# Bergvca/string_grouper

Measured on AMD Instinct MI355X. Metric: hot-path rows/sec (the device path of match_strings: tokenise + tf-idf + postings + SpGEMM-topn, inputs resident in HBM), 663k-name self-join ntop=10 min_sim=0.8; match_strings end to end: match_strings_rows_per_s, higher is better.
Workload: dtype f32

## Files before the change

string_grouper_amd/csrc/sg_spgemm_pruned.hip:

```cpp
#define SG_WATCH_NAME sg_debug_watch_pruned
#include "sg_k4_device.h"

#ifdef SG_DEBUG_WAVE_TIMES
__device__ unsigned long long sg_debug_wave_times[4 * 16384];
extern "C" int sg_debug_read_wave_times(unsigned long long *out, int clear) {
    if (hipMemcpyFromSymbol(out, HIP_SYMBOL(sg_debug_wave_times), sizeof(sg_debug_wave_times)) != hipSuccess) return 1;
    if (clear) {
        static unsigned long long zero[4 * 16384];
        if (hipMemcpyToSymbol(HIP_SYMBOL(sg_debug_wave_times), zero, sizeof(zero)) != hipSuccess) return 1;
    }
    return 0;
}
#endif

#ifndef SG_F64_STREAM_WAVES
#define SG_F64_STREAM_WAVES 4
#endif
#define SG_SCHED_FENCE() __builtin_amdgcn_sched_barrier(0)
#define SG_ROW_PARTS_LOG2 6
#define SG_ROW_PARTS 64u
#define SG_SURV_CAP 128

__device__ __forceinline__ uint64_t ballot64(bool p) { return __builtin_amdgcn_ballot_w64(p); }

template <typename T>
__device__ __forceinline__ T wave_shfl(T v, int src) {
    return __shfl(v, src, 64);
}

#define SG_HASH_SLOTS 128
#ifdef SG_HASH_FINE
__device__ __forceinline__ uint32_t term_hash(int k) { return (__umul24((uint32_t)k & 0xffffffu, 0x9E3779u) >> 15) & 127u; }
#else
__device__ __forceinline__ uint32_t term_hash(int k) { return (__umul24((uint32_t)k & 0xffffffu, 0x9E3779u) >> 15) & 124u; }
#endif

template <typename P>
__device__ __forceinline__ P *lds_object(uint32_t byte_addr) {
    typedef __attribute__((address_space(3))) P lds_t;
    return (P *)(lds_t *)(uintptr_t)byte_addr;
}

template <typename P>
__device__ __forceinline__ const __attribute__((address_space(1))) P *global_ptr(const void *p) {
    return (const __attribute__((address_space(1))) P *)(uintptr_t)p;
}
typedef uint32_t sg_u32x4 __attribute__((ext_vector_type(4)));
typedef uint32_t sg_u32x2 __attribute__((ext_vector_type(2)));
__device__ __forceinline__ uint4 load_global_u4(const void *base, size_t idx) {
    const sg_u32x4 v = global_ptr<sg_u32x4>(base)[idx];
    return make_uint4(v.x, v.y, v.z, v.w);
}
__device__ __forceinline__ uint2 load_global_u2(const void *base, size_t idx) {
    const sg_u32x2 v = global_ptr<sg_u32x2>(base)[idx];
    return make_uint2(v.x, v.y);
}

template <typename S>
__device__ __forceinline__ S load_launch_constants(const S *p) {
    static_assert(sizeof(S) % 4 == 0, "dwords");
    const uint64_t a = (uint64_t)(uintptr_t)p;
    const uint64_t u = ((uint64_t)(uint32_t)__builtin_amdgcn_readfirstlane((int)(uint32_t)(a >> 32)) << 32) |
                       (uint64_t)(uint32_t)__builtin_amdgcn_readfirstlane((int)(uint32_t)a);
    typedef const __attribute__((address_space(4))) uint32_t *const_words;
    const const_words w = (const_words)(uintptr_t)u;
    union {
        S s;
        uint32_t d[sizeof(S) / 4];
    } out = {};
#pragma unroll
    for (unsigned i = 0; i < sizeof(S) / 4; ++i) out.d[i] = w[i];
    return out.s;
}

template <typename T>
struct FwdRound;
template <>
struct FwdRound<float> {
    int k[8];
    float v[8];
    __device__ __forceinline__ void load(const void *fwd, uint32_t q, uint32_t last) {
#pragma unroll
        for (int e = 0; e < 4; ++e) {
            const uint4 w = load_global_u4(fwd, min((q >> 1) + e, last >> 1));
            k[2 * e] = (int)w.x;
            v[2 * e] = __uint_as_float(w.y);
            k[2 * e + 1] = (int)w.z;
            v[2 * e + 1] = __uint_as_float(w.w);
        }
    }
};
template <>
struct FwdRound<double> {
    int k[8];
    double v[8];
// ... 332 lines not shown
        c0 = surv[lane];
        k0 = (uint32_t)lane < n_clean ||
             __hip_atomic_exchange(&dt[((uint32_t)c0 * 2654435761u) >> 25], (uint32_t)c0, __ATOMIC_RELAXED,
                                   __HIP_MEMORY_SCOPE_WORKGROUP) != (uint32_t)c0;
    }
    if ((uint32_t)lane + 64u < n_surv) {
        c1 = surv[lane + 64];
        k1 = (uint32_t)lane + 64u < n_clean ||
             __hip_atomic_exchange(&dt[((uint32_t)c1 * 2654435761u) >> 25], (uint32_t)c1, __ATOMIC_RELAXED,
                                   __HIP_MEMORY_SCOPE_WORKGROUP) != (uint32_t)c1;
    }
    const uint64_t f0 = ballot64(k0), f1 = ballot64(k1);
    const uint32_t n0 = (uint32_t)__popcll(f0);
    __builtin_amdgcn_wave_barrier();
    if (k0) surv[__popcll(f0 & lanes_below)] = c0;
    if (k1) surv[n0 + __popcll(f1 & lanes_below)] = c1;
    __builtin_amdgcn_wave_barrier();
    FlushOut<T> out;
    out.top = top;
    out.n_surv = (uint32_t)__builtin_amdgcn_readfirstlane((int)(n0 + (uint32_t)__popcll(f1)));
    if (out.n_surv >= 63u) {
        out.top = drain_survivors<T, SYM, TILE_LOG2, WIDE, true>(nnz, thr, row, sc, pairs, top, out.n_surv);
        const uint32_t scored = out.n_surv < 64u ? out.n_surv : 64u;
        out.n_surv = (out.n_surv - scored) | (scored << 16);
    }
    return out;
}

template <typename T, int TILE_LOG2>
__device__ __noinline__ void emit_part_matches(const SgPairSink *__restrict__ pairs, T s, int c, int cnt, uint32_t row_out) {
    constexpr int TILE = 1 << TILE_LOG2;
    int *surv = lds_object<int>(TILE * 2 + 512 + 1024);
    const int lane = threadIdx.x;
    if (cnt <= 0) return;
    uint32_t pos = (uint32_t)surv[SG_SURV_CAP - 1];
    const SgPairSink pv = load_launch_constants(pairs);
    const uint32_t pair_chunks = pv.chunks;
    if (pos == SG_PAIR_NO_CHUNK || (pos & 511u) + (uint32_t)cnt > SG_PAIR_CHUNK) {
        uint32_t ch = 0;
        if (lane == 0) {
            if (pos != SG_PAIR_NO_CHUNK && (pos >> 9) < pair_chunks) {
                pv.d_chunk_count[pos >> 9] = pos & 511u;
                atomicAdd(pv.d_totals, (unsigned long long)(pos & 511u));
            }
            ch = atomicAdd(pv.d_chunks_used, 1u);
        }
        pos = (uint32_t)__builtin_amdgcn_readfirstlane((int)ch) << 9;
    }
    if ((pos >> 9) < pair_chunks) {
        if (lane < cnt) {
            const size_t o = (size_t)(pos >> 9) * SG_PAIR_CHUNK + (pos & 511u) + (uint32_t)lane;
            pv.d_i[o] = (uint32_t)c;
            pv.d_j[o] = row_out;
            reinterpret_cast<T *>(pv.d_s)[o] = s;
        }
        if (lane == 0) atomicAdd(&pv.d_row_count[row_out], (uint32_t)cnt);
    }
    __builtin_amdgcn_wave_barrier();
    if (lane == 0) surv[SG_SURV_CAP - 1] = (int)(pos + (uint32_t)cnt);
}

template <typename T, int TILE_LOG2, bool SYM, bool WIDE, int FOLD_LOG2, bool SHARE = false>
__global__ void __launch_bounds__(64, (sizeof(T) == 8 && FOLD_LOG2 > 0) ? SG_F64_STREAM_WAVES : 4)
spgemm_topn_pruned_kernel(const int64_t *__restrict__ a_indptr, const int32_t *__restrict__ a_indices,
                          const T *__restrict__ a_data, uint32_t n_left, const uint32_t *__restrict__ seg,
                          const uint32_t *__restrict__ ends, int32_t nt_pad, uint32_t n_terms,
                          const uint32_t *__restrict__ filt, int32_t n_tiles,
                          const SgScoreCtx *__restrict__ sc ,
                          int32_t keep, int32_t out_stride, T thr,
                          float s_budget , float norm_b ,
                          uint32_t freq_min ,
                          int32_t *__restrict__ out_cols, T *__restrict__ out_vals, int32_t *__restrict__ out_cnt,
                          uint32_t *row_counter, uint32_t *flagged_count, uint32_t *flagged_rows,
                          unsigned long long *stats ,
                          const SgPairSink *__restrict__ pairs ,
                          uint32_t pair_chunks ,
                          uint32_t sym_lo, uint32_t sym_hi ,
                          const uint32_t *__restrict__ row_list , const uint32_t *row_list_len,
                          const uint32_t *__restrict__ ends8 , int32_t nv_pad,
                          uint32_t null_off ,
                          uint32_t n_right ,
                          uint32_t *heavy_count, uint32_t *heavy_rows ,
                          uint32_t sym_step, uint32_t deal_floor ,
                          uint32_t part_cfg ) {
    constexpr int TILE = 1 << TILE_LOG2;
    constexpr int SLOTS = WIDE ? 2 : 1;
    constexpr int AB = TILE_LOG2 + 1;
    constexpr uint32_t ADDR_MASK = ((1u << AB) - 1u) & ~3u;
    constexpr int FB = AB + FOLD_LOG2;
    constexpr uint32_t BQ_BITS = 24 - FB;
    constexpr uint32_t BQ_MAX = (1u << BQ_BITS) - 1u;
    constexpr float SCALE = (float)(32768 >> FOLD_LOG2);
    extern __shared__ __attribute__((aligned(16))) unsigned char smem[];
    int *hk = reinterpret_cast<int *>(smem + TILE * 2);
    T *ha = reinterpret_cast<T *>(smem + TILE * 2 + 512);
    int *surv = reinterpret_cast<int *>(smem + TILE * 2 + 512 + 1024);
    uint4 *tab_v = reinterpret_cast<uint4 *>(smem);
    const int lane = threadIdx.x;
    for (int x = lane; x < TILE * 2 / 16; x += 64) tab_v[x] = make_uint4(0, 0, 0, 0);
    if (SYM && lane == 0) surv[SG_SURV_CAP - 1] = (int)SG_PAIR_NO_CHUNK;
    if (FOLD_LOG2 > 0 && lane == 0) surv[SG_SURV_CAP - 2] = 0;
    const uint64_t lanes_below = (1ull << lane) - 1ull;
    unsigned long long st_rows = 0, st_post = 0, st_surv = 0;
    auto tab_at = [&](uint32_t byte_addr) {
        typedef __attribute__((address_space(3))) uint32_t lds_u32;
        return (uint32_t *)(lds_u32 *)(uintptr_t)byte_addr;
    };
    auto filt_at = [&](uint32_t byte_off) {
        return *reinterpret_cast<const uint32_t *>(reinterpret_cast<const char *>(filt) + byte_off);
    };

    SG_WD_DECL(wd_rows);
    constexpr bool CAN_SPLIT = SYM && !WIDE && FOLD_LOG2 > 0 && SHARE;
    const bool part_mode = CAN_SPLIT && (part_cfg >> 31) != 0u;
#ifdef SG_DEBUG_WAVE_TIMES
    const unsigned long long dbg_t0 = __builtin_amdgcn_s_memrealtime();
    unsigned long long dbg_worst = 0, dbg_worst_row = 0;
#endif
    const uint32_t n_here = (WIDE || part_mode) ? (uint32_t)__builtin_amdgcn_readfirstlane((int)*row_list_len) << (part_mode ? SG_ROW_PARTS_LOG2 : 0)
                                                : (SYM ? (sym_hi - sym_lo + sym_step - 1u) / sym_step : n_left);
    const uint32_t n_single = min(n_here, 2u * gridDim.x);
    const uint32_t n_quads = (n_here - n_single) >> 2;
    for (uint32_t hlp = next_row(row_counter, lane);; hlp = next_row(row_counter, lane)) {
    const uint32_t row0 = hlp < n_quads ? hlp << 2 : (n_quads << 2) + (hlp - n_quads);
    if (row0 >= n_here || hlp >= 0x10000000u) break;
    for (uint32_t rr = row0; rr < row0 + (hlp < n_quads ? 4u : 1u); ++rr) {
        SG_WD(wd_rows, n_left + 2, 11)
        const uint32_t row = WIDE ? (uint32_t)__builtin_amdgcn_readfirstlane((int)row_list[rr])
                                  : part_mode ? (uint32_t)__builtin_amdgcn_readfirstlane((int)row_list[rr >> SG_ROW_PARTS_LOG2])
                                              : (SYM ? sym_hi - 1u - rr * sym_step : rr);
        uint32_t part_lo = 0, part_hi = 0;
        if (CAN_SPLIT && part_mode) {
            const uint32_t from = (uint32_t)__builtin_amdgcn_readfirstlane((int)row_list[n_left + (rr >> SG_ROW_PARTS_LOG2)]);
            const uint32_t nv = (((row >> TILE_LOG2) + (1u << FOLD_LOG2)) >> FOLD_LOG2) - from;
            const uint32_t part = rr & (SG_ROW_PARTS - 1u);
            part_lo = from + ((part * nv) >> SG_ROW_PARTS_LOG2);
            part_hi = from + (((part + 1u) * nv) >> SG_ROW_PARTS_LOG2);
            if (part_lo == part_hi) continue;
        }
        uint32_t row_out = row;
        if (SYM) {
            const uint32_t *orig_of = sc->orig_of;
            if (orig_of) row_out = (uint32_t)__builtin_amdgcn_readfirstlane((int)orig_of[row]);
        }
        const int64_t rlo = a_indptr[row];
        const int nnz = __builtin_amdgcn_readfirstlane((int)(a_indptr[row + 1] - rlo));
        if (nnz > 64 * SLOTS) {
            if (lane == 0) flagged_rows[atomicAdd(flagged_count, 1u)] = row;
            continue;
        }
        if (nnz == 0) continue;
        int k[SLOTS];
        T a[SLOTS], a2[SLOTS];
        uint32_t df[SLOTS], lo_e[SLOTS], key[SLOTS];
        float w[SLOTS], cum[SLOTS];
        uint64_t fm[SLOTS];
#pragma unroll
        for (int sl = 0; sl < SLOTS; ++sl) {
            k[sl] = 0;
            a[sl] = (T)0;
            df[sl] = lo_e[sl] = 0;
            const bool have = lane + 64 * sl < nnz;
            if (have) {
                k[sl] = a_indices[rlo + lane + 64 * sl];
                a[sl] = a_data[rlo + lane + 64 * sl];
                const uint32_t *sp = seg + (int64_t)k[sl] * n_tiles;
                lo_e[sl] = sp[0];
                df[sl] = sp[n_tiles] - lo_e[sl];
            }
            a2[sl] = mul_rn<T>(a[sl], a[sl]);
            w[sl] = have ? (sizeof(T) == 4 ? (float)a2[sl] : (float)a[sl] * (float)a[sl]) * 1.00001f : 0.f;
            cum[sl] = 0.f;
            key[sl] = (min(df[sl], (1u << 25) - 1u) << 7) | (127u - (uint32_t)(lane + 64 * sl));
            fm[sl] = ballot64(have && df[sl] >= freq_min);
        }
        const bool sum_own = SYM && FOLD_LOG2 > 0 && !part_mode;
        T own = (T)0;
        auto rank_step = [&](int sl_q, int f) {
            const uint32_t kq = wave_read<uint32_t>(key[sl_q], f);
            const float wq = wave_read<float>(w[sl_q], f);
#pragma unroll
            for (int sl = 0; sl < SLOTS; ++sl) cum[sl] += kq >= key[sl] ? wq : 0.f;
        };
        if (sum_own) {
#pragma unroll
            for (int sl_q = 0; sl_q < SLOTS; ++sl_q) {
                const int n_q = min(nnz - 64 * sl_q, 64);
                for (int f = 0; f < n_q; ++f) {
                    own = add_rn<T>(own, wave_read<T>(a2[sl_q], f));
                    if ((fm[sl_q] >> f) & 1ull) rank_step(sl_q, f);
                }
            }
        } else {
#pragma unroll
            for (int sl_q = 0; sl_q < SLOTS; ++sl_q) {
                uint64_t m = fm[sl_q];
                SG_WD_DECL(wd_r);
                while (m) {
                    SG_WD(wd_r, 70, 18)
                    const int f = __builtin_ctzll(m);
                    m &= m - 1;
                    rank_step(sl_q, f);
                }
            }
        }
        bool in_p[SLOTS];
        uint64_t pm[SLOTS];
        float bs2 = 0.f;
        uint32_t dsum_i = 0;
        int np = 0;
#pragma unroll
        for (int sl = 0; sl < SLOTS; ++sl) {
            const bool have = lane + 64 * sl < nnz;
            const bool in_s = have && cum[sl] <= s_budget && df[sl] >= freq_min;
            in_p[sl] = have && !in_s;
            pm[sl] = __ballot(in_p[sl]);
            np += __popcll(pm[sl]);
            bs2 = fmaxf(bs2, in_s ? cum[sl] : 0.f);
            dsum_i += in_p[sl] ? df[sl] : 0u;
        }
        if (np == 0) continue;
        if (np > 64) {
            if (lane == 0) flagged_rows[atomicAdd(flagged_count, 1u)] = row;
            continue;
        }
        if (!part_mode) ++st_rows;
#ifdef SG_DEBUG_WAVE_TIMES
        const unsigned long long dbg_r0 = __builtin_amdgcn_s_memrealtime();
        const unsigned long long dbg_surv0 = st_surv;
#endif
#pragma unroll
        for (int d = 32; d > 0; d >>= 1) {
            bs2 = fmaxf(bs2, __shfl_xor(bs2, d, 64));
            dsum_i += __shfl_xor(dsum_i, d, 64);
        }
        bs2 = wave_read<float>(bs2, 0);
        dsum_i = wave_read<uint32_t>(dsum_i, 0);
        if (dsum_i == 0u) continue;
        const float b_s = sqrtf(bs2) * 1.000002f;
        const float t0 = ((float)thr - 1e-5f) * SCALE - 2.0f;
        const float c1 = b_s * norm_b * (SCALE / 255.0f) * 1.000002f;
        const int32_t T0 = (int32_t)floorf(t0 * 256.0f) - 256 * np;
        const int32_t C1 = (int32_t)(c1 * 256.0f) + 1;
        const int32_t C16 = (int32_t)(b_s * norm_b * (SCALE * 65536.0f / 65280.0f) * 1.000002f) + 1;
        const int32_t T16 = T0 << 8;
        const int32_t T0s = T16 - 32768 * C16, C1n = -C16;
        if (FOLD_LOG2 > 0 ? !(T16 - C16 * 65535 >= 65536) : !(T0 - C1 * 255 >= 256)) {
            if (lane == 0) flagged_rows[atomicAdd(flagged_count, 1u)] = row;
            continue;
        }
        const int32_t T0m = T0 - 256;

        uint32_t G[SLOTS], rem[SLOTS];
#pragma unroll
        for (int sl = 0; sl < SLOTS; ++sl) {
            rem[sl] = 0u;
            if (deal_floor) {
                G[sl] = in_p[sl] ? sg_deal_floor_rule(df[sl], (float)dsum_i, np) : 0u;
// ... 143 lines not shown
                old = __hip_atomic_fetch_add(tab_at(zaddr), xs, __ATOMIC_RELAXED, __HIP_MEMORY_SCOPE_WORKGROUP);
            asm volatile("" : "+v"(old));
            const uint32_t oh = __builtin_amdgcn_ubfe(old, sh, 16u);
            const uint64_t cm = ballot64(tq1 - oh < x) & valid_mask;
            if (cm) collect(cm, r, t);
        };

        struct Batch {
            uint32_t r0, r1, r2, r3;
            int32_t rem;
            uint32_t base;
        };
        auto issue = [&](Batch &bt, uint32_t lo, uint32_t hi) {
            bt.base = lo + u16;
            bt.rem = (int32_t)(hi - bt.base);
            struct __attribute__((packed, aligned(4))) Quad {
                uint32_t x, y, z, w;
            };
            const Quad q = *reinterpret_cast<const Quad *>(reinterpret_cast<const char *>(filt) + bt.base);
            bt.r0 = q.x;
            bt.r1 = q.y;
            bt.r2 = q.z;
            bt.r3 = q.w;
        };
        struct Slot {
            uint32_t z, sh, x, xs, tq1;
        };
        auto prep = [&](uint32_t r) {
            Slot s;
            s.z = r & ADDR_MASK;
            s.sh = r << 4;
            s.x = (uint32_t)(((uint64_t)(r & (BQ_MAX << FB)) * (uint64_t)(CA & 0xffffffu)) >> 32);
            s.tq1 = (uint32_t)((T0m - __mul24(C1, (int32_t)(r >> 24))) >> 8);
            asm("v_lshlrev_b32 %0, %1, %2" : "=v"(s.xs) : "v"(s.sh), "v"(s.x));
            return s;
        };
        auto apply = [&](const Batch &bt, uint32_t t) {
            const bool v0 = bt.rem > 0, v1 = bt.rem > 4, v2 = bt.rem > 8, v3 = bt.rem > 12;
            const uint64_t m0 = ballot64(v0), m1 = ballot64(v1), m2 = ballot64(v2), m3 = ballot64(v3);
            if (m0 == 0) return;
            if (ballot64(bt.rem > over16)) {
                uint32_t zz = 0;
                round(bt.r0, v0, m0, t, zz);
                round(bt.r1, v1, m1, t, zz);
                round(bt.r2, v2, m2, t, zz);
                round(bt.r3, v3, m3, t, zz);
                int32_t left = bt.rem - over16 - (int32_t)u4;
                uint32_t at = bt.base + (uint32_t)over16 + u4;
                SG_WD_DECL(wd_b);
                uint64_t ml;
                while ((ml = ballot64(left > 0)) != 0) {
                    SG_WD(wd_b, 1 << 24, 14)
                    const uint32_t rx = filt_at(at);
                    round(rx, left > 0, ml, t, zz);
                    left -= (int32_t)G4;
                    at += G4;
                }
                for (int x = lane; x < TILE * 2 / 16; x += 64) tab_v[x] = make_uint4(0, 0, 0, 0);
                return;
            }
            const Slot s0 = prep(bt.r0), s1 = prep(bt.r1), s2 = prep(bt.r2), s3 = prep(bt.r3);
            const uint32_t a0 = v0 ? s0.xs : 0u, a1 = v1 ? s1.xs : 0u, a2 = v2 ? s2.xs : 0u, a3 = v3 ? s3.xs : 0u;
            uint32_t o0 = __hip_atomic_fetch_add(tab_at(s0.z), a0, __ATOMIC_RELAXED, __HIP_MEMORY_SCOPE_WORKGROUP);
            uint32_t o1 = __hip_atomic_fetch_add(tab_at(s1.z), a1, __ATOMIC_RELAXED, __HIP_MEMORY_SCOPE_WORKGROUP);
            uint32_t o2 = __hip_atomic_fetch_add(tab_at(s2.z), a2, __ATOMIC_RELAXED, __HIP_MEMORY_SCOPE_WORKGROUP);
            uint32_t o3 = __hip_atomic_fetch_add(tab_at(s3.z), a3, __ATOMIC_RELAXED, __HIP_MEMORY_SCOPE_WORKGROUP);
            *tab_at(s0.z) = 0u;
            *tab_at(s1.z) = 0u;
            *tab_at(s2.z) = 0u;
            *tab_at(s3.z) = 0u;
            asm volatile("" : "+v"(o0), "+v"(o1), "+v"(o2), "+v"(o3));
            const uint64_t c0 = ballot64(s0.tq1 - __builtin_amdgcn_ubfe(o0, s0.sh, 16u) < s0.x) & m0;
            const uint64_t c1m = ballot64(s1.tq1 - __builtin_amdgcn_ubfe(o1, s1.sh, 16u) < s1.x) & m1;
            const uint64_t c2 = ballot64(s2.tq1 - __builtin_amdgcn_ubfe(o2, s2.sh, 16u) < s2.x) & m2;
            const uint64_t c3 = ballot64(s3.tq1 - __builtin_amdgcn_ubfe(o3, s3.sh, 16u) < s3.x) & m3;
            if (c0 | c1m | c2 | c3) {
                if (c0) collect(c0, bt.r0, t);
                if (c1m) collect(c1m, bt.r1, t);
                if (c2) collect(c2, bt.r2, t);
                if (c3) collect(c3, bt.r3, t);
            }
        };

        if constexpr (FOLD_LOG2 == 0) {
            uint4 E0 = ends_at(0);
            uint4 E1 = ends_at(min(1u, last_group));
            const uint32_t list_lo = g ? my_lo << 2 : 0u;
            Batch b0, b1, b2, b3;
            issue(b0, list_lo, E0.x);
            issue(b1, E0.x, E0.y);
            issue(b2, E0.y, E0.z);
            SG_WD_DECL(wd_t);
            for (uint32_t t = 0; t < t_end; t += 4) {
                SG_WD(wd_t, n_tiles + 2, 13)
                const uint4 E2 = ends_at(min((t >> 2) + 2u, last_group));
                issue(b3, E0.z, E0.w);
                apply(b0, t);
                if (t + 1 >= t_end) break;
                issue(b0, E0.w, E1.x);
                apply(b1, t + 1);
                if (t + 2 >= t_end) break;
                issue(b1, E1.x, E1.y);
                apply(b2, t + 2);
                if (t + 3 >= t_end) break;
                issue(b2, E1.y, E1.z);
                apply(b3, t + 3);
                E0 = E1;
                E1 = E2;
            }
        } else {
            constexpr int FOLD = 1 << FOLD_LOG2;
            constexpr uint32_t COL_MASK = (1u << (TILE_LOG2 + FOLD_LOG2)) - 1u;
            uint32_t *dt = reinterpret_cast<uint32_t *>(smem + TILE * 2 + 512 + (sizeof(T) == 4 ? 512 : 1024 + SG_SURV_CAP * 4));
            dt[lane] = 0xFFFFFFFFu;
            dt[lane + 64] = 0xFFFFFFFFu;
            const uint32_t n_visits = (t_end + (uint32_t)FOLD - 1u) >> FOLD_LOG2;
            const uint32_t erow8 = (g ? (uint32_t)my_k : n_terms) * (uint32_t)nv_pad;
            auto ends8_at = [&](uint32_t group) {
                return *reinterpret_cast<const uint4 *>(reinterpret_cast<const char *>(ends8) + ((erow8 + (group << 2)) << 2));
            };
            const uint32_t last_group8 = (uint32_t)(nv_pad >> 2) - 1u;
            const uint32_t hi_end = ends[(size_t)erow + t_end - 1u];
            typedef uint32_t u32x4 __attribute__((ext_vector_type(4)));
            uint32_t v_lo = 0, v_end = n_visits;
            uint32_t hi_stop = hi_end;
            uint32_t cur = (g ? my_lo << 2 : 0u) + u16;
            if (CAN_SPLIT) {
                if (part_mode) {
                    v_lo = part_lo;
                    v_end = part_hi;
                    const uint32_t *e8 = ends8 + erow8;
                    if (v_end < n_visits) hi_stop = min(hi_end, e8[v_end - 1u]);
                    if (v_lo) cur = e8[v_lo - 1u] + u16;
                } else if (part_cfg != 0u && n_visits >= 2u) {
                    float rl = g ? (float)(hi_end - (my_lo << 2)) / (float)G16 : 0.f;
#pragma unroll
                    for (int d = 32; d > 0; d >>= 1) rl = fmaxf(rl, __shfl_xor(rl, d, 64));
                    if (wave_read<float>(rl, 0) >= (float)(part_cfg & 0x0fffffffu)) {
                        if (lane == 0) {
                            const uint32_t at = atomicAdd(heavy_count, 1u);
                            heavy_rows[at] = row;
                            heavy_rows[n_left + at] = 0u;
                        }
                        continue;
                    }
                }
            }
            uint32_t row_scored = 0;
            asm volatile("" : "+v"(row_scored));
            u32x4 EA, EB;
            {
                const uint32_t g0 = v_lo >> 2;
                const uint4 a = ends8_at(g0), b = ends8_at(min(g0 + 1u, last_group8));
                const u32x4 av = u32x4{a.x, a.y, a.z, a.w}, bv = u32x4{b.x, b.y, b.z, b.w};
                EA = (g0 & 1u) ? bv : av;
                EB = (g0 & 1u) ? av : bv;
            }
            auto end_of_visit = [&](uint32_t v) {
                const uint32_t c = v & 3u;
                const uint32_t ea = c == 0 ? EA.x : (c == 1 ? EA.y : (c == 2 ? EA.z : EA.w));
                const uint32_t eb = c == 0 ? EB.x : (c == 1 ? EB.y : (c == 2 ? EB.z : EB.w));
                return (v & 4u) ? eb : ea;
            };
            const uint32_t erow8_b = erow8 << 2;
            auto load_ends = [&](uint32_t sel, uint32_t grp) {
                uint32_t e_off;
                asm volatile(
                    "s_cmp_gt_u32 %[sel], 1\n\t"
                    "s_cbranch_scc1 .Lends_done%=\n\t"
                    "v_lshl_add_u32 %[off], %[grp], 4, %[erow]\n\t"
                    "s_cmp_eq_u32 %[sel], 0\n\t"
                    "s_cbranch_scc0 .Lends_b%=\n\t"
                    "global_load_dwordx4 %[EA], %[off], %[base]\n\t"
                    "s_branch .Lends_done%=\n"
                    ".Lends_b%=:\n\t"
                    "global_load_dwordx4 %[EB], %[off], %[base]\n"
                    ".Lends_done%=:"
                    : [EA] "+v"(EA), [EB] "+v"(EB), [off] "=&v"(e_off)
                    : [sel] "s"(sel), [grp] "s"(grp), [erow] "v"(erow8_b), [base] "s"(ends8)
                    : "scc", "memory");
            };
            uint32_t gv = v_lo;
            uint32_t hi = min(end_of_visit(v_lo), hi_stop);

            struct SBatch {
                u32x4 q;
            };
            const uint32_t null_at = null_off + ((uint32_t)lane << 4);
            bool live = hi > cur;
            auto issue_s = [&](SBatch &bt, uint32_t &tv, bool &last) {
                tv = gv;
                {
                    const uint32_t at = live ? cur : null_at;
                    asm volatile("global_load_dwordx4 %0, %1, %2" : "+v"(bt.q) : "v"(at), "s"(filt) : "memory");
                }
                cur += G16;
                live = hi > cur;
                last = ballot64(live) == 0;
                uint32_t sel = 2u, grp = 0u;
                if (last) {
                    ++gv;
                    if ((gv & 3u) == 0u) {
                        grp = min((gv >> 2) + 1u, last_group8);
                        sel = ((gv >> 2) + 1u) & 1u;
                    }
// ... 10 lines not shown
                asm volatile("s_waitcnt vmcnt(0) ; rounds %0 %1 %2 ends %3 %4" : "+v"(oa.q), "+v"(ob.q), "+v"(oc.q), "+v"(EA), "+v"(EB)::"memory");
                const FlushOut<T> fo = flush_survivors<T, SYM, TILE_LOG2, WIDE>(nnz, thr, row_arg, sc, pairs, top, n_surv, n_clean);
                top = fo.top;
                const uint32_t fo_word = (uint32_t)__builtin_amdgcn_readfirstlane((int)fo.n_surv);
                st_surv += fo_word >> 16;
                if (CAN_SPLIT) {
                    row_scored += fo_word >> 16;
                    if (!part_mode && part_cfg != 0u && tv + 3u <= v_end && ballot64((uint64_t)row_scored >= ((uint64_t)(part_cfg & 0x0fffffffu) << ((part_cfg >> 28) & 7u))) != 0) v_end = tv + 1u;
                }
                n_surv = n_clean = fo_word & 0xffffu;
            };
            auto collect_s = [&](bool fired, uint64_t cm, uint32_t r, uint32_t tv, SBatch &oa, SBatch &ob, SBatch &oc) {
                const uint32_t col = (tv << (TILE_LOG2 + FOLD_LOG2)) | ((r >> 1) & COL_MASK);
                const bool mine = SYM ? col <= row : col < n_right;
                cm &= ballot64(mine);
                const uint32_t n_new = (uint32_t)__popcll(cm);
                if (n_surv + n_new > (uint32_t)SG_SURV_CAP - 2u) flush_s(oa, ob, oc, tv);
                const uint32_t below = __builtin_amdgcn_mbcnt_hi((uint32_t)(cm >> 32), __builtin_amdgcn_mbcnt_lo((uint32_t)cm, 0u));
                if (fired && mine) surv[n_surv + below] = (int)col;
                n_surv += n_new;
            };
            struct SSlot {
                uint32_t z, sh, xs, x;
                uint32_t d;
            };
            auto prep_s = [&](uint32_t r) {
                SSlot q;
                q.z = r & ADDR_MASK;
                q.sh = r << 3;
                q.x = (uint32_t)(((uint64_t)(r & 0xffffffu) * (uint64_t)(CA & 0xffffffu)) >> 32);
                asm("v_lshlrev_b32 %0, %1, %2" : "=v"(q.xs) : "v"(q.sh), "v"(q.x));
                q.d = 0;
                return q;
            };
            auto bar_s = [&](uint32_t r) {
                uint32_t d;
                asm("v_mad_i32_i16 %0, %1, %2, %3 op_sel:[1,0,0,0]" : "=v"(d) : "v"(r), "v"(C1n), "v"(T0s));
                return d;
            };
            bool dirty = false;
            auto apply_s = [&](SBatch &bt, SBatch &oa, SBatch &ob, SBatch &oc, uint32_t tv, bool last) {
                asm volatile("s_waitcnt vmcnt(3) ; round %0" : "+v"(bt.q)::"memory");
                const u32x4 q = bt.q;
                {
                    dirty = true;
                    SSlot s0 = prep_s(q.x);
                    uint32_t o0 = __hip_atomic_fetch_add(tab_at(s0.z), s0.xs, __ATOMIC_RELAXED, __HIP_MEMORY_SCOPE_WORKGROUP);
                    SG_SCHED_FENCE();
                    SSlot s1 = prep_s(q.y);
                    uint32_t o1 = __hip_atomic_fetch_add(tab_at(s1.z), s1.xs, __ATOMIC_RELAXED, __HIP_MEMORY_SCOPE_WORKGROUP);
                    SG_SCHED_FENCE();
                    SSlot s2 = prep_s(q.z);
                    uint32_t o2 = __hip_atomic_fetch_add(tab_at(s2.z), s2.xs, __ATOMIC_RELAXED, __HIP_MEMORY_SCOPE_WORKGROUP);
                    SG_SCHED_FENCE();
                    SSlot s3 = prep_s(q.w);
                    uint32_t o3 = __hip_atomic_fetch_add(tab_at(s3.z), s3.xs, __ATOMIC_RELAXED, __HIP_MEMORY_SCOPE_WORKGROUP);
                    SG_SCHED_FENCE();
                    s0.d = bar_s(q.x);
                    s1.d = bar_s(q.y);
                    s2.d = bar_s(q.z);
                    s3.d = bar_s(q.w);
                    asm volatile("" : "+v"(s0.d), "+v"(s1.d), "+v"(s2.d), "+v"(s3.d));
                    asm volatile("" : "+v"(o0), "+v"(o1), "+v"(o2), "+v"(o3));
                    const bool f0 = ((__builtin_amdgcn_ubfe(o0, s0.sh, 16u) + s0.x) << 16) >= s0.d;
                    const bool f1 = ((__builtin_amdgcn_ubfe(o1, s1.sh, 16u) + s1.x) << 16) >= s1.d;
                    const bool f2 = ((__builtin_amdgcn_ubfe(o2, s2.sh, 16u) + s2.x) << 16) >= s2.d;
                    const bool f3 = ((__builtin_amdgcn_ubfe(o3, s3.sh, 16u) + s3.x) << 16) >= s3.d;
                    const uint64_t c0 = ballot64(f0), c1m = ballot64(f1), c2 = ballot64(f2), c3 = ballot64(f3);
                    if (c0 | c1m | c2 | c3) {
                        if (c0) collect_s(f0, c0, q.x, tv, oa, ob, oc);
                        if (c1m) collect_s(f1, c1m, q.y, tv, oa, ob, oc);
                        if (c2) collect_s(f2, c2, q.z, tv, oa, ob, oc);
                        if (c3) collect_s(f3, c3, q.w, tv, oa, ob, oc);
                    }
                }
                if (last && dirty) {
#pragma unroll
                    for (int x = 0; x < TILE * 2 / 16; x += 64) tab_v[x + lane] = make_uint4(0, 0, 0, 0);
                    dirty = false;
                }
            };
            uint32_t tv0, tv1, tv2, tv3;
            bool la0, la1, la2, la3;
            issue_s(sb0, tv0, la0);
            issue_s(sb1, tv1, la1);
            issue_s(sb2, tv2, la2);
            issue_s(sb3, tv3, la3);
            SG_WD_DECL(wd_s);
            for (;;) {
                SG_WD(wd_s, 1 << 26, 17)
                if (tv0 >= v_end) break;
                apply_s(sb0, sb1, sb2, sb3, tv0, la0);
                issue_s(sb0, tv0, la0);
                if (tv1 >= v_end) break;
                apply_s(sb1, sb2, sb3, sb0, tv1, la1);
                issue_s(sb1, tv1, la1);
                if (tv2 >= v_end) break;
                apply_s(sb2, sb3, sb0, sb1, tv2, la2);
                issue_s(sb2, tv2, la2);
                if (tv3 >= v_end) break;
                apply_s(sb3, sb0, sb1, sb2, tv3, la3);
                issue_s(sb3, tv3, la3);
            }
            asm volatile("s_waitcnt vmcnt(0) ; rounds %0 %1 %2 %3 ends %4 %5" : "+v"(sb0.q), "+v"(sb1.q), "+v"(sb2.q), "+v"(sb3.q), "+v"(EA), "+v"(EB)::"memory");
            if (n_surv > n_clean) flush_s(sb1, sb2, sb3, v_end);
            if (CAN_SPLIT && !part_mode && v_end != n_visits && lane == 0) {
                const uint32_t at = atomicAdd(heavy_count, 1u);
                heavy_rows[at] = row;
                heavy_rows[n_left + at] = v_end;
            }
        }
        {
            uint32_t mine = 0;
            if (g && u == 0 && part_lo == 0u) {
                const uint32_t *erp = ends + (size_t)erow;
                mine = (erp[t_end - 1u] >> 2) - my_lo;
            }
#pragma unroll
            for (int d = 32; d > 0; d >>= 1) mine += __shfl_xor(mine, d, 64);
            st_post += (unsigned long long)wave_read<uint32_t>(mine, 0);
        }
        if (n_surv > 0) {
            top = drain_survivors<T, SYM, TILE_LOG2, WIDE, (FOLD_LOG2 > 0)>(nnz, thr, row_arg, sc, pairs, top, n_surv);
            st_surv += n_surv;
        }
        if (CAN_SPLIT && part_mode) {
            int cnt = __popcll(__ballot(top.c != INT32_MAX));
            if (cnt > keep) cnt = keep;
            emit_part_matches<T, TILE_LOG2>(pairs, top.s, top.c, cnt, row_out);
        } else {
            int cnt = __popcll(__ballot(top.c != INT32_MAX));
            if (cnt > keep) cnt = keep;
            const size_t obase = (size_t)row_out * (size_t)out_stride;
            if (lane < cnt) {
                out_vals[obase + lane] = top.s;
                out_cols[obase + lane] = top.c;
            }
            if (lane == 0) out_cnt[row_out] = cnt;
        }
        if (SYM) {
            const uint32_t pos = (uint32_t)__builtin_amdgcn_readfirstlane(surv[SG_SURV_CAP - 1]);
            if (pos != SG_PAIR_NO_CHUNK && (pos >> 9) >= pair_chunks && lane == 0) atomicMax(row_counter, 0x20000000u);
        }
#ifdef SG_DEBUG_WAVE_TIMES
        {
            const unsigned long long dt = __builtin_amdgcn_s_memrealtime() - dbg_r0;
            if (dt > dbg_worst) {
                dbg_worst = dt;
                dbg_worst_row = (unsigned long long)row | ((st_surv - dbg_surv0) << 32);
            }
        }
#endif
    }
    }
    if (SYM && lane == 0) {
        const uint32_t pos = (uint32_t)surv[SG_SURV_CAP - 1];
        if (pos != SG_PAIR_NO_CHUNK && (pos >> 9) < pair_chunks) {
            pairs->d_chunk_count[pos >> 9] = pos & 511u;
            atomicAdd(pairs->d_totals, (unsigned long long)(pos & 511u));
        }
    }
    if (lane == 0) {
        if (st_rows) atomicAdd(stats + 0, st_rows);
        if (st_post) atomicAdd(stats + 1, st_post);
        if (st_surv) atomicAdd(stats + 2, st_surv);
        if (FOLD_LOG2 > 0) {
            if (surv[SG_SURV_CAP - 2]) atomicAdd(stats + 4, (unsigned long long)(uint32_t)surv[SG_SURV_CAP - 2]);
        } else if (st_surv) atomicAdd(stats + 4, st_surv);
    }
#ifdef SG_DEBUG_WAVE_TIMES
    if (SYM && !WIDE && FOLD_LOG2 > 0 && sizeof(T) == 4 && lane == 0 && blockIdx.x < 8192u) {
        unsigned long long *w = sg_debug_wave_times + 4u * (blockIdx.x + (part_mode ? 8192u : 0u));
        w[0] = dbg_t0;
        w[1] = __builtin_amdgcn_s_memrealtime();
        w[2] = dbg_worst;
        w[3] = dbg_worst_row;
    }
#endif
}

extern "C" int sg_debug_deal_lanes(const uint32_t *df, int np, uint32_t *G_out, int floor_rule) {
    if (np < 1 || np > 64 || !df || !G_out) return 1;
    uint64_t dsum = 0;
    for (int t = 0; t < np; ++t) dsum += df[t];
    if (dsum == 0) return 1;
    if (floor_rule) {
        for (int t = 0; t < np; ++t) G_out[t] = sg_deal_floor_rule(df[t], (float)dsum, np);
        return 0;
    }
    const uint32_t spare = (uint32_t)(64 - np);
    uint64_t rem[64];
    uint32_t given = 0;
    for (int t = 0; t < np; ++t) {
        uint32_t q = 0;
        sg_deal_share<uint64_t>(df[t], dsum, spare, q, rem[t]);
        if (dsum < (1ull << 30)) {
            uint32_t q32 = 0, rem32 = 0;
            sg_deal_share<uint32_t>(df[t], (uint32_t)dsum, spare, q32, rem32);
            if (q32 != q || rem32 != rem[t]) return 2;
        }
        G_out[t] = 1u + q;
        given += G_out[t];
    }
    if (given < 64u) {
        const uint32_t R = 64u - given;
        const uint64_t cut = sg_deal_cut<uint64_t>(dsum, R, [&](uint64_t c) {
            uint32_t n = 0;
            for (int t = 0; t < np; ++t) n += rem[t] >= c ? 1u : 0u;
            return n;
        });
        uint32_t left = R;
        for (int t = 0; t < np; ++t)
            if (rem[t] > cut) {
                ++G_out[t];
                --left;
            }
        for (int t = 0; t < np && left; ++t)
            if (rem[t] == cut) {
                ++G_out[t];
                --left;
            }
    }
    return 0;
}

__device__ __forceinline__ void publish_pass_stats(const unsigned long long *src, const uint32_t *word, unsigned long long *dst) {
    if (dst != nullptr && blockIdx.x == 0 && threadIdx.x == 0) {
        dst[0] = src[0];
        dst[1] = src[1];
        dst[2] = src[2];
        dst[4] = src[4];
        reinterpret_cast<uint32_t *>(dst + 3)[0] = *word;
    }
}

template <typename T>
__global__ void __launch_bounds__(SG_PAIR_CHUNK) pairs_fill_kernel(const uint32_t *__restrict__ pi, const uint32_t *__restrict__ pj,
                                                                   const T *__restrict__ ps, const uint32_t *__restrict__ chunk_count,
                                                                   const uint32_t *__restrict__ ptr, uint32_t *cursor,
                                                                   int32_t *__restrict__ lcol, T *__restrict__ lval) {
    if (threadIdx.x >= chunk_count[blockIdx.x]) return;
    const size_t p = (size_t)blockIdx.x * SG_PAIR_CHUNK + threadIdx.x;
    const uint32_t j = pj[p];
    const uint32_t at = ptr[j] + atomicAdd(&cursor[j], 1u);
    lcol[at] = (int32_t)pi[p];
    lval[at] = ps[p];
}

template <typename T>
__global__ void __launch_bounds__(SG_PAIR_CHUNK) pairs_export_kernel(const uint32_t *__restrict__ pi, const uint32_t *__restrict__ pj,
                                                                     const T *__restrict__ ps, const uint32_t *__restrict__ chunk_count,
                                                                     const uint32_t *__restrict__ chunk_start, int32_t *__restrict__ out,
// ... 278 lines not shown
struct PairList {
    SgPairSink sink;
    const SgPairSink *d_sink = nullptr;
    uint32_t row_lo = 0, row_hi = 0;
    uint32_t row_step = 1;
    uint32_t rows() const { return (row_hi - row_lo + row_step - 1u) / row_step; }
};

__global__ void pair_sink_kernel(SgPairSink v, SgPairSink *out) { *out = v; }

bool sg_q8_applies(const sg_ctx *ctx, const sg_postings *Bt, double threshold) {
    if (!Bt->d_q8 || Bt->fold_log2 <= 0) return false;
    return threshold >= ctx->opt_double("SG_Q8_MIN_THRESHOLD", 0.65);
}

static size_t pruned_lds(int32_t tile_log2, int32_t fold_log2, int32_t dtype) {
    return ((size_t)2 << tile_log2) + 512 + 1024 + (size_t)SG_SURV_CAP * 4 + (fold_log2 > 0 && dtype == SG_F64 ? 512 : 0);
}
static unsigned pruned_grid(const sg_ctx *ctx, int32_t tile_log2, int64_t n_rows, int32_t fold_log2 = 0, int32_t dtype = SG_F32) {
    const size_t lds = pruned_lds(tile_log2, fold_log2, dtype);
    int waves_per_cu = (int)(ctx->lds_per_cu / lds);
    if (waves_per_cu > 32) waves_per_cu = 32;
    if (waves_per_cu < 1) waves_per_cu = 1;
    const int forced = ctx->opt_int("SG_PRUNE_WAVES_PER_CU", 0);
    if (forced > 0) waves_per_cu = forced;
    unsigned grid = (unsigned)ctx->num_cu * (unsigned)waves_per_cu;
    if ((int64_t)grid > n_rows) grid = (unsigned)(n_rows > 0 ? n_rows : 1);
    return grid;
}

struct PrunedJob {
    sg_ctx *ctx;
    const sg_csr *A;
    const sg_postings *Bt;
    int32_t keep;
    sg_topn *r;
    double threshold;
    float s_budget;
    unsigned long long *stats = nullptr;
    uint32_t *row_counter = nullptr;
    uint32_t *flagged_count = nullptr, *flagged_rows = nullptr;
    const PairList *pl = nullptr;
};

struct PrunedLaunch {
    uint32_t *row_counter;
    uint32_t *out_count, *out_rows;
    const uint32_t *in_rows = nullptr, *in_len = nullptr;
    uint32_t *heavy_count = nullptr, *heavy_rows = nullptr;
    uint32_t part_cfg = 0;
};

struct RowList {
    uint32_t *base = nullptr;
    uint32_t *count() const { return base; }
    uint32_t *counter() const { return base ? base + 1 : nullptr; }
    uint32_t *rows() const { return base ? base + 4 : nullptr; }
};

template <typename T, int TILE_LOG2, bool SYM, bool WIDE, int FOLD_LOG2>
static int launch_pruned(const PrunedJob &job, const PrunedLaunch &l) {
    sg_ctx *ctx = job.ctx;
    const sg_csr *A = job.A;
    const sg_postings *Bt = job.Bt;
    const sg_topn *r = job.r;
    const PairList &pl = *job.pl;
    const T thr = (T)job.threshold;
    const size_t lds = pruned_lds(TILE_LOG2, FOLD_LOG2, A->dtype);
    unsigned grid = pruned_grid(ctx, TILE_LOG2, SYM ? (int64_t)pl.rows() : A->n_rows, FOLD_LOG2, A->dtype);
    if (WIDE && grid > (unsigned)ctx->num_cu * 4u && (double)A->nnz <= 48.0 * (double)A->n_rows) grid = (unsigned)ctx->num_cu * 4u;
    constexpr bool SPLITS = SYM && !WIDE && FOLD_LOG2 > 0;
    const bool share = SPLITS && (l.heavy_count != nullptr || l.part_cfg != 0u);
    auto kernel = share ? spgemm_topn_pruned_kernel<T, TILE_LOG2, SYM, WIDE, FOLD_LOG2, SPLITS>
                        : spgemm_topn_pruned_kernel<T, TILE_LOG2, SYM, WIDE, FOLD_LOG2, false>;
    hipLaunchKernelGGL(kernel, dim3(grid), dim3(64), lds, ctx->stream, A->d_indptr,
                       A->d_indices, (const T *)A->d_data, (uint32_t)A->n_rows, (const uint32_t *)Bt->d_seg,
                       (const uint32_t *)Bt->d_ends, Bt->nt_pad, (uint32_t)Bt->n_terms,
                       (const uint32_t *)Bt->d_filt, Bt->n_tiles,
                       (const SgScoreCtx *)Bt->d_score_ctx + (sg_q8_applies(ctx, Bt, (double)thr) ? 0 : 1), job.keep, r->stride, thr,
                       job.s_budget, Bt->norm_up, Bt->freq_min, r->d_cols,
                       (T *)r->d_vals,
                       r->d_counts, l.row_counter, l.out_count, l.out_rows, job.stats, pl.d_sink, pl.sink.chunks, pl.row_lo, pl.row_hi,
                       l.in_rows, l.in_len, (const uint32_t *)Bt->d_ends8, Bt->nv_pad, (uint32_t)(Bt->nnz * 4), (uint32_t)Bt->n_right,
                       l.heavy_count, l.heavy_rows, pl.row_step, ctx->opt_is("SG_DEAL", 'f') ? 1u : 0u, l.part_cfg);
    SG_HIP_TRY(hipGetLastError());
    return SG_OK;
}

static uint32_t heavy_part_cfg(const sg_ctx *ctx, const sg_csr *A, const PairList &range, int32_t tile_log2, int32_t fold_log2) {
    uint32_t heavy_rounds = 0;
    if ((range.row_lo > 0 || (int64_t)range.row_hi < A->n_rows || range.row_step > 1) && 2 * (int64_t)range.rows() < A->n_rows) {
        const double n_idx = (double)A->n_rows;
        const double rows_per_wave = (double)range.rows() / (double)pruned_grid(ctx, tile_log2, (int64_t)range.rows(), fold_log2, A->dtype);
        const double rounds_per_row = 2.0 * 7.2e-5 * n_idx * (0.5 * ((double)range.row_lo + (double)range.row_hi) / n_idx);
        const double share = ctx->opt_double("SG_HEAVY_SHARE", 0.0);
        const double bar_share = share > 0.0 ? share : 0.05;
        const double bar = bar_share * rows_per_wave * rounds_per_row;
        heavy_rounds = bar < 128.0 ? 128u : (bar > 1.0e9 ? 1000000000u : (uint32_t)bar);
    }
    heavy_rounds = (uint32_t)ctx->opt_int("SG_HEAVY_ROUNDS", (int)heavy_rounds) & 0x7fffffffu;
    if (heavy_rounds > 0x0fffffffu) heavy_rounds = 0x0fffffffu;
    uint32_t handover_shift = heavy_rounds >= 512u ? 1u : (heavy_rounds >= 256u ? 2u : 3u);
    handover_shift = (uint32_t)ctx->opt_int("SG_HANDOVER_SHIFT", (int)handover_shift) & 7u;
    if (heavy_rounds) heavy_rounds |= handover_shift << 28;
    return heavy_rounds;
}

template <typename T, int TILE_LOG2, bool SYM, int FOLD_LOG2>
static int launch_both(const PrunedJob &job) {
    sg_ctx *ctx = job.ctx;
    const int64_t n_rows = job.A->n_rows;
    Scratch scratch(ctx);
    RowList l1, heavy;
    SG_TRY(scratch.alloc((size_t)n_rows + 8, &l1.base));
    if (hipMemsetAsync(l1.base, 0, 4 * sizeof(uint32_t), ctx->stream) != hipSuccess) return SG_ERR_HIP;
    uint32_t part_cfg = 0;
    if (SYM && FOLD_LOG2 > 0) part_cfg = heavy_part_cfg(ctx, job.A, *job.pl, TILE_LOG2, FOLD_LOG2);
    if (part_cfg) {
        SG_TRY(scratch.alloc(2 * (size_t)n_rows + 8, &heavy.base));
        if (hipMemsetAsync(heavy.base, 0, 4 * sizeof(uint32_t), ctx->stream) != hipSuccess) return SG_ERR_HIP;
    }
    const PrunedLaunch first{job.row_counter, l1.count(), l1.rows(), nullptr, nullptr, heavy.count(), heavy.rows(), part_cfg};
    SG_TRY((launch_pruned<T, TILE_LOG2, SYM, false, FOLD_LOG2>(job, first)));
    if (heavy.base) {
        const PrunedLaunch parts{heavy.counter(), l1.count(), l1.rows(), heavy.rows(), heavy.count(), nullptr, nullptr, 0x80000000u};
        SG_TRY((launch_pruned<T, TILE_LOG2, SYM, false, FOLD_LOG2>(job, parts)));
        scratch.release(heavy.base);
    }
    if (!ctx->opt_is("SG_PRUNE_WIDE", '0')) {
        const PrunedLaunch wide{l1.counter(), job.flagged_count, job.flagged_rows, l1.rows(), l1.count()};
        return launch_pruned<T, TILE_LOG2, SYM, true, FOLD_LOG2>(job, wide);
    }
    if (hipMemcpyAsync(job.flagged_count, l1.count(), 4, hipMemcpyDeviceToDevice, ctx->stream) != hipSuccess ||
        hipMemcpyAsync(job.flagged_rows, l1.rows(), sizeof(uint32_t) * (size_t)n_rows, hipMemcpyDeviceToDevice, ctx->stream) != hipSuccess)
        return SG_ERR_HIP;
    return SG_OK;
}

template <typename T, bool SYM>
static int dispatch_pruned(const PrunedJob &job) {
    const sg_postings *Bt = job.Bt;
    if (Bt->fold_log2 > 0) {
        if (Bt->fold_log2 != 3 || Bt->tile_log2 != 12 || !Bt->d_ends8) {
            sg_set_error("postings folded 2^%d over tiles of 2^%d columns are not supported by the pruned multiply", Bt->fold_log2,
                         Bt->tile_log2);
            return SG_ERR_UNSUPPORTED;
        }
        return launch_both<T, 12, SYM, 3>(job);
    }
    switch (Bt->tile_log2) {
        case 11: return launch_both<T, 11, SYM, 0>(job);
        case 12: return launch_both<T, 12, SYM, 0>(job);
        case 13: return launch_both<T, 13, SYM, 0>(job);
        default:
            sg_set_error("postings tile of 2^%d columns is not supported by the pruned multiply (2^11..2^13)", Bt->tile_log2);
            return SG_ERR_UNSUPPORTED;
    }
}

bool sg_pruned_supports_tile(int32_t tile_log2) { return tile_log2 >= 11 && tile_log2 <= 13; }

static float prune_budget(const sg_postings *Bt, double threshold, double delta) {
    const double nb = (double)Bt->norm_up;
    const double beta = threshold - delta;
    const double budget = (beta / nb) * (beta / nb) * (1.0 - 1e-6);
    return __builtin_nextafterf((float)budget, 0.f);
}
// ... 280 lines not shown
```

Baseline: 108.0 million.

## Prefetch next row's indices and postings bounds during current row's stream

In the symmetric folded non-shared kernel, the wave now issues loads for the next row (row-1): its indptr, indices, values and orig_of entry. These are issued after the current row's streaming loop and before the final vmcnt wait, and the seg lo/hi bounds are fetched once the wait completes. The next row then takes these from registers via lane shuffles instead of reloading them, hiding the per-row load latency. The stored stream end is also reused so the ends entry is not read a second time. The change adds register pressure and relies on rows within a quad being contiguous and descending. Default-off debug phase timers are added as well.

```diff
diff --git a/string_grouper_amd/csrc/sg_spgemm_pruned.hip b/string_grouper_amd/csrc/sg_spgemm_pruned.hip
--- a/string_grouper_amd/csrc/sg_spgemm_pruned.hip
+++ b/string_grouper_amd/csrc/sg_spgemm_pruned.hip
@@ -11,6 +11,30 @@
     }
     return 0;
 }
+#endif
+#ifdef SG_DEBUG_ROW_PHASES
+__device__ uint32_t sg_debug_row_phases[16 * 8192];
+extern "C" int sg_debug_read_row_phases(uint32_t *out, int clear) {
+    if (hipMemcpyFromSymbol(out, HIP_SYMBOL(sg_debug_row_phases), sizeof(sg_debug_row_phases)) != hipSuccess) return 1;
+    if (clear) {
+        static uint32_t zero[16 * 8192];
+        if (hipMemcpyToSymbol(HIP_SYMBOL(sg_debug_row_phases), zero, sizeof(zero)) != hipSuccess) return 1;
+    }
+    return 0;
+}
+__device__ __forceinline__ uint32_t phase_clock_s(uint32_t dep) {
+    unsigned long long t;
+    asm volatile("s_memrealtime %0\n\ts_waitcnt lgkmcnt(0)" : "=s"(t) : "s"(dep) : "memory");
+    return (uint32_t)t;
+}
+__device__ __forceinline__ uint32_t phase_clock_v(uint32_t dep0, uint32_t dep1) {
+    unsigned long long t;
+    asm volatile("s_memrealtime %0\n\ts_waitcnt lgkmcnt(0)" : "=s"(t) : "v"(dep0), "v"(dep1) : "memory");
+    return (uint32_t)t;
+}
+#define SG_PHASE(var, expr) var = (expr)
+#else
+#define SG_PHASE(var, expr)
 #endif
 
 #ifndef SG_F64_STREAM_WAVES
@@ -509,7 +533,8 @@
                           uint32_t n_right ,
                           uint32_t *heavy_count, uint32_t *heavy_rows ,
                           uint32_t sym_step, uint32_t deal_floor ,
-                          uint32_t part_cfg ) {
+                          uint32_t part_cfg ,
+                          uint32_t row_ahead ) {
     constexpr int TILE = 1 << TILE_LOG2;
     constexpr int SLOTS = WIDE ? 2 : 1;
     constexpr int AB = TILE_LOG2 + 1;
@@ -548,11 +573,41 @@
                                                 : (SYM ? (sym_hi - sym_lo + sym_step - 1u) / sym_step : n_left);
     const uint32_t n_single = min(n_here, 2u * gridDim.x);
     const uint32_t n_quads = (n_here - n_single) >> 2;
-    for (uint32_t hlp = next_row(row_counter, lane);; hlp = next_row(row_counter, lane)) {
+    constexpr bool PIPE = SYM && !WIDE && FOLD_LOG2 > 0 && !SHARE;
+    const bool do_ahead = PIPE && row_ahead != 0u && sym_step == 1u;
+    bool ah_have = false;
+    int64_t ah_rlo = 0;
+    int ah_nnz = 0;
+    uint32_t ah_row_out = 0;
+    int ah_k = 0;
+    T ah_a = (T)0;
+    uint32_t ah_lo = 0, ah_hi = 0;
+#ifdef SG_DEBUG_ROW_PHASES
+    const uint32_t ph_born = phase_clock_s(0u);
+    uint32_t ph_ticket = 0, ph_tickets = 0, ph_begun = 0, ph_done = 0, ph_loads = 0, ph_rank = 0, ph_ends = 0, ph_first = 0, ph_rounds = 0,
+             ph_tail = 0;
+    auto take_ticket = [&]() {
+        const uint32_t t = phase_clock_s(0u);
+        const uint32_t h = next_row(row_counter, lane);
+        ph_ticket += phase_clock_s(h) - t;
+        ++ph_tickets;
+        return h;
+    };
+#define SG_TAKE_TICKET() take_ticket()
+#else
+#define SG_TAKE_TICKET() next_row(row_counter, lane)
+#endif
+    for (uint32_t hlp = SG_TAKE_TICKET();; hlp = SG_TAKE_TICKET()) {
     const uint32_t row0 = hlp < n_quads ? hlp << 2 : (n_quads << 2) + (hlp - n_quads);
     if (row0 >= n_here || hlp >= 0x10000000u) break;
-    for (uint32_t rr = row0; rr < row0 + (hlp < n_quads ? 4u : 1u); ++rr) {
+    const uint32_t hlp_end = row0 + (hlp < n_quads ? 4u : 1u);
+    for (uint32_t rr = row0; rr < hlp_end; ++rr) {
         SG_WD(wd_rows, n_left + 2, 11)
+#ifdef SG_DEBUG_ROW_PHASES
+        uint32_t ph_t1 = 0, ph_t2 = 0, ph_t3 = 0, ph_t4 = 0, ph_t5 = 0;
+        const uint32_t ph_t0 = phase_clock_s(rr);
+        ++ph_begun;
+#endif
         const uint32_t row = WIDE ? (uint32_t)__builtin_amdgcn_readfirstlane((int)row_list[rr])
                                   : part_mode ? (uint32_t)__builtin_amdgcn_readfirstlane((int)row_list[rr >> SG_ROW_PARTS_LOG2])
                                               : (SYM ? sym_hi - 1u - rr * sym_step : rr);
@@ -566,12 +621,22 @@
             if (part_lo == part_hi) continue;
         }
         uint32_t row_out = row;
-        if (SYM) {
-            const uint32_t *orig_of = sc->orig_of;
-            if (orig_of) row_out = (uint32_t)__builtin_amdgcn_readfirstlane((int)orig_of[row]);
-        }
-        const int64_t rlo = a_indptr[row];
-        const int nnz = __builtin_amdgcn_readfirstlane((int)(a_indptr[row + 1] - rlo));
+        int64_t rlo;
+        int nnz;
+        const bool ahead = PIPE && ah_have;
+        if (PIPE && ahead) {
+            ah_have = false;
+            row_out = ah_row_out;
+            rlo = ah_rlo;
+            nnz = ah_nnz;
+        } else {
+            if (SYM) {
+                const uint32_t *orig_of = sc->orig_of;
+                if (orig_of) row_out = (uint32_t)__builtin_amdgcn_readfirstlane((int)orig_of[row]);
+            }
+            rlo = a_indptr[row];
+            nnz = __builtin_amdgcn_readfirstlane((int)(a_indptr[row + 1] - rlo));
+        }
         if (nnz > 64 * SLOTS) {
             if (lane == 0) flagged_rows[atomicAdd(flagged_count, 1u)] = row;
             continue;
@@ -588,7 +653,18 @@
             a[sl] = (T)0;
             df[sl] = lo_e[sl] = 0;
             const bool have = lane + 64 * sl < nnz;
-            if (have) {
+            if (PIPE && ahead) {
+                const int from = nnz - 1 - lane;
+                const int qk = wave_shfl<int>(ah_k, from);
+                const T qa = wave_shfl<T>(ah_a, from);
+                const uint32_t qlo = wave_shfl<uint32_t>(ah_lo, from), qhi = wave_shfl<uint32_t>(ah_hi, from);
+                if (have) {
+                    k[sl] = qk;
+                    a[sl] = qa;
+                    lo_e[sl] = qlo;
+                    df[sl] = qhi - qlo;
+                }
+            } else if (have) {
                 k[sl] = a_indices[rlo + lane + 64 * sl];
                 a[sl] = a_data[rlo + lane + 64 * sl];
                 const uint32_t *sp = seg + (int64_t)k[sl] * n_tiles;
@@ -601,6 +677,7 @@
             key[sl] = (min(df[sl], (1u << 25) - 1u) << 7) | (127u - (uint32_t)(lane + 64 * sl));
             fm[sl] = ballot64(have && df[sl] >= freq_min);
         }
+        SG_PHASE(ph_t1, phase_clock_v(df[0], __float_as_uint(w[0])));
         const bool sum_own = SYM && FOLD_LOG2 > 0 && !part_mode;
         T own = (T)0;
         auto rank_step = [&](int sl_q, int f) {
@@ -910,6 +987,7 @@
             }
         };
 
+        uint32_t stream_end = 0;
         if constexpr (FOLD_LOG2 == 0) {
             uint4 E0 = ends_at(0);
             uint4 E1 = ends_at(min(1u, last_group));
@@ -948,7 +1026,9 @@
                 return *reinterpret_cast<const uint4 *>(reinterpret_cast<const char *>(ends8) + ((erow8 + (group << 2)) << 2));
             };
             const uint32_t last_group8 = (uint32_t)(nv_pad >> 2) - 1u;
+            SG_PHASE(ph_t2, phase_clock_v(erow8, CA));
             const uint32_t hi_end = ends[(size_t)erow + t_end - 1u];
+            stream_end = hi_end;
             typedef uint32_t u32x4 __attribute__((ext_vector_type(4)));
             uint32_t v_lo = 0, v_end = n_visits;
             uint32_t hi_stop = hi_end;
@@ -1125,10 +1205,15 @@
             };
             uint32_t tv0, tv1, tv2, tv3;
             bool la0, la1, la2, la3;
+            SG_PHASE(ph_t3, phase_clock_v(hi, cur));
             issue_s(sb0, tv0, la0);
             issue_s(sb1, tv1, la1);
             issue_s(sb2, tv2, la2);
             issue_s(sb3, tv3, la3);
+#ifdef SG_DEBUG_ROW_PHASES
+            asm volatile("s_waitcnt vmcnt(3) ; round %0" : "+v"(sb0.q)::"memory");
+            ph_t4 = phase_clock_s(0u);
+#endif
             SG_WD_DECL(wd_s);
             for (;;) {
                 SG_WD(wd_s, 1 << 26, 17)
@@ -1145,7 +1230,36 @@
                 apply_s(sb3, sb0, sb1, sb2, tv3, la3);
                 issue_s(sb3, tv3, la3);
             }
+            if constexpr (PIPE) {
+                if (do_ahead && rr + 1u < hlp_end) {
+                    const int64_t at = rlo - 1 - (int64_t)lane;
+                    ah_k = 0;
+                    ah_a = (T)0;
+                    if (at >= 0) {
+                        ah_k = a_indices[at];
+                        ah_a = a_data[at];
+                    }
+                    ah_rlo = a_indptr[row - 1u];
+                    ah_row_out = row - 1u;
+                    const uint32_t *orig_of = sc->orig_of;
+                    if (orig_of) ah_row_out = orig_of[row - 1u];
+                    ah_have = true;
+                }
+            }
             asm volatile("s_waitcnt vmcnt(0) ; rounds %0 %1 %2 %3 ends %4 %5" : "+v"(sb0.q), "+v"(sb1.q), "+v"(sb2.q), "+v"(sb3.q), "+v"(EA), "+v"(EB)::"memory");
+            SG_PHASE(ph_t5, phase_clock_s(0u));
+            if constexpr (PIPE) {
+                if (ah_have) {
+                    ah_row_out = (uint32_t)__builtin_amdgcn_readfirstlane((int)ah_row_out);
+                    ah_nnz = __builtin_amdgcn_readfirstlane((int)(rlo - ah_rlo));
+                    ah_lo = ah_hi = 0;
+                    if (ah_nnz <= 64 && lane < ah_nnz) {
+                        const uint32_t *sp = seg + (int64_t)ah_k * n_tiles;
+                        ah_lo = sp[0];
+                        ah_hi = sp[n_tiles];
+                    }
+                }
+            }
             if (n_surv > n_clean) flush_s(sb1, sb2, sb3, v_end);
             if (CAN_SPLIT && !part_mode && v_end != n_visits && lane == 0) {
                 const uint32_t at = atomicAdd(heavy_count, 1u);
@@ -1156,8 +1270,11 @@
         {
             uint32_t mine = 0;
             if (g && u == 0 && part_lo == 0u) {
-                const uint32_t *erp = ends + (size_t)erow;
-                mine = (erp[t_end - 1u] >> 2) - my_lo;
+                if constexpr (FOLD_LOG2 > 0 && !CAN_SPLIT) mine = (stream_end >> 2) - my_lo;
+                else {
+                    const uint32_t *erp = ends + (size_t)erow;
+                    mine = (erp[t_end - 1u] >> 2) - my_lo;
+                }
             }
 #pragma unroll
             for (int d = 32; d > 0; d >>= 1) mine += __shfl_xor(mine, d, 64);
@@ -1185,6 +1302,18 @@
             const uint32_t pos = (uint32_t)__builtin_amdgcn_readfirstlane(surv[SG_SURV_CAP - 1]);
             if (pos != SG_PAIR_NO_CHUNK && (pos >> 9) >= pair_chunks && lane == 0) atomicMax(row_counter, 0x20000000u);
         }
+#ifdef SG_DEBUG_ROW_PHASES
+        if (FOLD_LOG2 > 0) {
+            const uint32_t ph_t6 = phase_clock_s(0u);
+            ++ph_done;
+            ph_loads += ph_t1 - ph_t0;
+            ph_rank += ph_t2 - ph_t1;
+            ph_ends += ph_t3 - ph_t2;
+            ph_first += ph_t4 - ph_t3;
+            ph_rounds += ph_t5 - ph_t4;
+            ph_tail += ph_t6 - ph_t5;
+        }
+#endif
 #ifdef SG_DEBUG_WAVE_TIMES
         {
             const unsigned long long dt = __builtin_amdgcn_s_memrealtime() - dbg_r0;
@@ -1211,6 +1340,15 @@
             if (surv[SG_SURV_CAP - 2]) atomicAdd(stats + 4, (unsigned long long)(uint32_t)surv[SG_SURV_CAP - 2]);
         } else if (st_surv) atomicAdd(stats + 4, st_surv);
     }
+#ifdef SG_DEBUG_ROW_PHASES
+    if (SYM && !WIDE && FOLD_LOG2 > 0 && sizeof(T) == 4 && !part_mode && lane == 0 && blockIdx.x < 8192u) {
+        uint32_t *w = sg_debug_row_phases + 16u * blockIdx.x;
+        const uint32_t v[11] = {ph_ticket, ph_tickets, ph_begun, ph_done, ph_loads, ph_rank, ph_ends, ph_first, ph_rounds, ph_tail,
+                                phase_clock_s(0u) - ph_born};
+#pragma unroll
+        for (int i = 0; i < 11; ++i) w[i] += v[i];
+    }
+#endif
 #ifdef SG_DEBUG_WAVE_TIMES
     if (SYM && !WIDE && FOLD_LOG2 > 0 && sizeof(T) == 4 && lane == 0 && blockIdx.x < 8192u) {
         unsigned long long *w = sg_debug_wave_times + 4u * (blockIdx.x + (part_mode ? 8192u : 0u));
@@ -1655,7 +1793,8 @@
                        (T *)r->d_vals,
                        r->d_counts, l.row_counter, l.out_count, l.out_rows, job.stats, pl.d_sink, pl.sink.chunks, pl.row_lo, pl.row_hi,
                        l.in_rows, l.in_len, (const uint32_t *)Bt->d_ends8, Bt->nv_pad, (uint32_t)(Bt->nnz * 4), (uint32_t)Bt->n_right,
-                       l.heavy_count, l.heavy_rows, pl.row_step, ctx->opt_is("SG_DEAL", 'f') ? 1u : 0u, l.part_cfg);
+                       l.heavy_count, l.heavy_rows, pl.row_step, ctx->opt_is("SG_DEAL", 'f') ? 1u : 0u, l.part_cfg,
+                       ctx->opt_int("SG_ROW_AHEAD", 1) != 0 ? 1u : 0u);
     SG_HIP_TRY(hipGetLastError());
     return SG_OK;
 }
```

After: 107.3 million. About the same (-0.7%).
